# adamgreig/labrador-ldpc

Hardware: AMD Instinct MI355X
Metric: decoded codewords/sec @25 min-sum iters, TM8192, Eb/N0=2dB; 1/2/4/8 GPU (higher is better)
Workload: dtype f32; 1 GPU; TM8192 f32 LLRs, 4194304 frames on 1 GPU = BASELINE config 4 whole, resident in HBM, max_iters 25 with early termination, AWGN Eb/N0 2.0 dB, 256 random codewords; code=TM8192, total_frames=4194304, frames_per_gpu=4194304, max_iters=25, parallelism=1 contiguous shard(s) of one batch, one process per GPU, no collective, kernel_variant=0, library_build=bc9a2135c5c5dfc7

## Files before the change

### labrador_ldpc_amd/csrc/decode_ms_pair.hpp

```cpp
#pragma once

#include "decode_ms_kernel.hpp"


namespace ldpc {


typedef float ldpc_f2 __attribute__((ext_vector_type(2)));

template <int CODE, class T>
struct PairGeometry {
    static constexpr int M = CODES[CODE].m;
    static constexpr int NT = M / 2;
    static constexpr int NX = count_exchanged(*CODES[CODE].proto);
    static constexpr int NXC = count_exch_cols(*CODES[CODE].proto);
    static constexpr int OUT_LEN = CODES[CODE].output_len();
    static constexpr int LDS_BYTES = ((NX + NXC) * M * 4 + 16 + 15) / 16 * 16;
    static_assert(M % 512 == 0 && NT <= 1024, "pair ownership needs M/8 >= 64 lanes per quarter and <= 1024 threads");
};

constexpr int pair_local_rank(const Prototype &p, int S, int B)
{
    int nloc = 0, r = 0;
    for (int b = 0; b < p.n_blocks; ++b)
        if (blk_local(p.blk[b])) { if (b < B) ++r; ++nloc; }
    return S * nloc + r;
}

constexpr bool all_exchanged_are_pi(const Prototype &p)
{
    for (int b = 0; b < p.n_blocks; ++b)
        if (!blk_local(p.blk[b]) && p.blk[b].kind != BLK_P) return false;
    return true;
}

template <class T, bool SOFT, bool CORRECTED>
constexpr int pair_hoist_addresses()
{
    if (LDPC_PAIR_HOIST >= 0) return LDPC_PAIR_HOIST;
    return (std::is_same_v<T, float> && !SOFT && !CORRECTED) ? LDPC_PAIR_HOIST_F32 : 0;
}

template <int CODE, class T, int JW, int FORM, bool SOFT = false, bool CORRECTED = false>
LDPC_DEV void decode_ms_pair_body(const T *__restrict__ llrs, uint8_t *__restrict__ output,
                                  uint32_t *__restrict__ iters_out, uint8_t *__restrict__ success_out,
                                  uint32_t batch, uint32_t maxiters, float nocap_limit, uint32_t *claim, char *lds,
                                  T *__restrict__ app = nullptr, float corr_scale = 1.0f, float corr_offset = 0.0f)
{
    static_assert(!CORRECTED || std::is_same_v<T, float>, "the correction step is built for f32 messages");
    using GEO = PairGeometry<CODE, T>;
    using O = Ops<T>;
    using R = typename O::R;
    static_assert(sizeof(R) == 4 && sizeof(typename O::E) == 4, "pair kernel: 4-byte message types");
    constexpr Prototype P = *CODES[CODE].proto;
    static_assert(all_exchanged_are_pi(P), "pair kernel: exchanged blocks must be pi_k");
    constexpr int M = GEO::M, NT = GEO::NT, NB = P.n_blocks, NROWS = P.n_rows, NCOLS = P.n_cols;
    constexpr int N = CODES[CODE].n, NTX = N / M, NX = GEO::NX, NXC = GEO::NXC;
    constexpr int Q = M / 4, IPT = 2;
    constexpr int BLK_BYTES = M * 4, FLAG_OFF = (NX + NXC) * BLK_BYTES;
    constexpr bool ODD_B64 = LDPC_PAIR_ODD_B64 >= 0 ? LDPC_PAIR_ODD_B64 != 0 : true;
    constexpr int LOCAL_IN_VAR = LDPC_PAIR_LOCAL_IN_VAR >= 0 ? LDPC_PAIR_LOCAL_IN_VAR : (std::is_same_v<T, float> ? 10 : 8);
    constexpr int HOIST = pair_hoist_addresses<T, SOFT, CORRECTED>();
    constexpr bool PRIO_WAVES = true;
    (void)PRIO_WAVES;

    const int t = (int)(threadIdx.x & (M / 8 - 1)) + JW * (M / 8);
    __builtin_assume(t >= 0 && t < NT);
    const uint32_t n_groups = batch;
    uint32_t cw = blockIdx.x;
    bool live = cw < batch;
    (void)live;

    auto lds1 = [&](int off) LDPC_INLINE -> float & { return *reinterpret_cast<float *>(lds + off); };
    auto lds2 = [&](int off) LDPC_INLINE -> ldpc_f2 & { return *reinterpret_cast<ldpc_f2 *>(lds + off); };
    auto flag_at = [&](uint32_t which) LDPC_INLINE -> int & { return *reinterpret_cast<int *>(lds + FLAG_OFF + 4 * (which & 1)); };
    auto cap_flag = [&]() LDPC_INLINE -> int & { return *reinterpret_cast<int *>(lds + FLAG_OFF + 8); };
    constexpr bool NOCAP_POSSIBLE = LDPC_PAIR_NOCAP && std::is_same_v<T, float>;

    auto even_c = [](int B) constexpr { return (phi_of(P.blk[B].val, JW, M) & 1) == 0; };
    auto wire = [&](auto B_, auto S_, int tb8) LDPC_INLINE -> int {
        constexpr int B = decltype(B_)::value, S = decltype(S_)::value;
        constexpr int K = P.blk[B].val;
        constexpr int base = (((theta_of(K) + JW) & 3) * Q) * 4 + lds_bias(P, B, BLK_BYTES);
        return ((tb8 + (phi_of(K, JW, M) + S) * 4) & (Q * 4 - 1)) | base;
    };

    R u[IPT][NB], v[IPT][NB], va[IPT][NCOLS], llr[IPT][NTX];
    T lraw[IPT][NTX];

    auto fetch_llrs = [&](uint32_t c) LDPC_INLINE {
        unsigned tu = (unsigned)t;
        asm volatile("" : "+v"(tu));
        const uint32_t cc = c < batch ? c : batch - 1;
        static_for<0, NTX>([&](auto C_) LDPC_INLINE {
            constexpr int C = decltype(C_)::value;
            const T *src = (llrs + (size_t)cc * N) + (unsigned)(C * M);
            lraw[0][C] = src[2 * tu];
            lraw[1][C] = src[2 * tu + 1];
        });
    };

    auto forget_llrs = [&]() LDPC_INLINE {
        static_for<0, IPT>([&](auto S_) LDPC_INLINE {
            static_for<0, NTX>([&](auto C_) LDPC_INLINE {
                if constexpr (sizeof(T) == 4) { T &x = lraw[decltype(S_)::value][decltype(C_)::value]; asm volatile("" : "=v"(x)); }
            });
        });
    };
    (void)forget_llrs;
    constexpr int VB_HI = 0x10000;
    int had[IPT][NB], vb[2];
    (void)had; (void)vb;
    auto hoist_addresses = [&]() LDPC_INLINE {
        int tq = t;
        asm volatile("" : "+v"(tq));
        const int tb8 = tq * 8;
        vb[0] = tb8;
        asm volatile("" : "+v"(vb[0]));
        if constexpr (FLAG_OFF > VB_HI) {
            vb[1] = tb8 + VB_HI;
            asm volatile("" : "+v"(vb[1]));
        }
        static_for<0, NB>([&](auto B_) LDPC_INLINE {
            constexpr int B = decltype(B_)::value;
            if constexpr (exch_slot(P, B) >= 0) {
                constexpr int lo = lds_bias(P, B, BLK_BYTES);
                static_assert(lds_xu_off(P, exch_slot(P, B), BLK_BYTES) - lo + 4 < 0x10000 && lds_xva_off(P, col_slot(P, P.blk[B].col), BLK_BYTES) - lo + 4 < 0x10000);
                if constexpr (even_c(B)) {
                    had[0][B] = wire(B_, IC<0>{}, tb8);
                } else if constexpr (ODD_B64) {
                    had[0][B] = wire(B_, IC<-1>{}, tb8);
                    had[1][B] = wire(B_, IC<1>{}, tb8);
                    asm volatile("" : "+v"(had[1][B]));
                } else {
                    had[0][B] = wire(B_, IC<0>{}, tb8);
                    had[1][B] = wire(B_, IC<1>{}, tb8);
                    asm volatile("" : "+v"(had[1][B]));
                }
                asm volatile("" : "+v"(had[0][B]));
            }
        });
    };
    auto own = [&](auto OFF_) LDPC_INLINE -> int {
        constexpr int off = decltype(OFF_)::value;
        if constexpr (off < VB_HI) return vb[0] + off;
        else return vb[1] + (off - VB_HI);
    };
    (void)own;

    auto begin_codeword = [&]() LDPC_INLINE {
        if constexpr (HOIST == 1) hoist_addresses();
        int tq = t;
        asm volatile("" : "+v"(tq));
        const int tb8 = tq * 8;
        static_for<0, IPT>([&](auto S_) LDPC_INLINE {
            constexpr int S = decltype(S_)::value;
            static_for<0, NB>([&](auto B_) LDPC_INLINE {
                constexpr int B = decltype(B_)::value;
                u[S][B] = O::zero();
                v[S][B] = O::zero();
            });
            static_for<0, NCOLS>([&](auto C_) LDPC_INLINE { va[S][decltype(C_)::value] = O::zero(); });
            static_for<0, NTX>([&](auto C_) LDPC_INLINE { llr[S][decltype(C_)::value] = O::load(lraw[S][decltype(C_)::value]); });
        });
        if constexpr (!LDPC_PAIR_PEEL_FIRST)
        static_for<0, NX>([&](auto X_) LDPC_INLINE {
            lds2(lds_xu_off(P, decltype(X_)::value, BLK_BYTES) + tb8) = ldpc_f2{0.0f, 0.0f};
        });
        if (t < 2) flag_at(t) = 0;
        if constexpr (NOCAP_POSSIBLE) {
            bool big = false;
            static_for<0, IPT>([&](auto S_) LDPC_INLINE {
                static_for<0, NTX>([&](auto C_) LDPC_INLINE {
                    const R a = O::mag(llr[decltype(S_)::value][decltype(C_)::value]);
                    big |= !(a <= nocap_limit) || (a != 0.0f && a < 0x1p-20f);
                });
            });
            if (__ballot(big) != 0 && (t & 63) == 0) cap_flag() = 1;
        }
    };

    auto edge_update = [&](auto S_, auto B_, R x, auto BND_) LDPC_INLINE {
        constexpr int S = decltype(S_)::value, B = decltype(B_)::value;
        const R nv = O::sub_nv(x, u[S][B]);
        constexpr bool BND = decltype(BND_)::value != 0;
        constexpr int F = (FORM >= 2 && (BND || sizeof(T) <= 2)) ? FORM : (LDPC_PAIR_SELFCORR_CARRY != 0 ? 1 : 0);
        v[S][B] = O::template self_correct_b<BND, F>(nv, v[S][B]);
    };

    auto variable_phase = [&](auto BND_, auto FIRST_) LDPC_INLINE {
        constexpr bool FIRST = decltype(FIRST_)::value != 0;
        int tq = t;
        if constexpr (HOIST == 0) asm volatile("" : "+v"(tq));
        const int tb8 = tq * 8;
        (void)tb8;
        LDPC_SETPRIO(LDPC_PRIO_VAR);
        static_for<0, NCOLS>([&](auto C_) LDPC_INLINE {
            constexpr int C = decltype(C_)::value;
            if constexpr (C == NCOLS / 2) LDPC_SETPRIO(0);
            R acc0 = O::zero(), acc1 = O::zero();
            if constexpr (C < NTX) { acc0 = llr[0][C]; acc1 = llr[1][C]; }
            if constexpr (!FIRST)
            static_for<0, NB>([&](auto B_) LDPC_INLINE {
                constexpr int B = decltype(B_)::value;
                if constexpr (P.blk[B].col == C) {
                    constexpr int slot = exch_slot(P, B);
                    if constexpr (slot >= 0) {
                        ldpc_f2 up;
                        if constexpr (HOIST != 0) up = lds2(own(IC<lds_xu_off(P, slot, BLK_BYTES)>{}));
                        else up = lds2(lds_xu_off(P, slot, BLK_BYTES) + tb8);
                        acc0 = O::add(acc0, O::from_lds(up.x));
                        acc1 = O::add(acc1, O::from_lds(up.y));
                    } else {
                        acc0 = O::add(acc0, u[0][B]);
                        acc1 = O::add(acc1, u[1][B]);
                    }
                }
            });
            va[0][C] = acc0;
            va[1][C] = acc1;
            constexpr int cs = col_slot(P, C);
            if constexpr (cs >= 0) {
                if constexpr (HOIST != 0) lds2(own(IC<lds_xva_off(P, cs, BLK_BYTES)>{})) = ldpc_f2{O::store(acc0), O::store(acc1)};
                else lds2(lds_xva_off(P, cs, BLK_BYTES) + tb8) = ldpc_f2{O::store(acc0), O::store(acc1)};
            }
        });
        static_for<0, IPT>([&](auto S_) LDPC_INLINE {
            static_for<0, NB>([&](auto B_) LDPC_INLINE {
                constexpr int S = decltype(S_)::value, B = decltype(B_)::value;
                if constexpr (exch_slot(P, B) < 0 && pair_local_rank(P, S, B) < LOCAL_IN_VAR) {
                    if constexpr (FIRST) v[S][B] = va[S][P.blk[B].col];
                    else edge_update(S_, B_, va[S][P.blk[B].col], BND_);
                }
            });
        });
    };

    auto check_phase = [&](uint32_t it, auto CAP_, auto FIRST_) LDPC_INLINE {
        constexpr bool CAP = decltype(CAP_)::value != 0;
        constexpr bool FIRST = decltype(FIRST_)::value != 0;
        constexpr int BND = (!CAP && NOCAP_POSSIBLE) ? 1 : 0;
        int par_any = 0;
        int tq = t;
        if constexpr (HOIST == 0) asm volatile("" : "+v"(tq));
        const int tb8 = tq * 8;
        (void)tb8;
        LDPC_SETPRIO(3);
        R xs[IPT][NB];
        int ad[IPT][NB];
        auto request_marginals = [&]() LDPC_INLINE {
        static_for<0, NB>([&](auto B_) LDPC_INLINE {
            constexpr int B = decltype(B_)::value;
            constexpr int slot = exch_slot(P, B);
            if constexpr (slot >= 0) {
                constexpr int cs = col_slot(P, P.blk[B].col);
                constexpr int off = lds_xva_off(P, cs, BLK_BYTES) - lds_bias(P, B, BLK_BYTES);
                if constexpr (HOIST != 0) {
                    ad[0][B] = had[0][B];
                    if constexpr (!even_c(B)) ad[1][B] = had[1][B];
                }
                if constexpr (even_c(B)) {
                    if constexpr (HOIST == 0) ad[0][B] = wire(B_, IC<0>{}, tb8);
                    const ldpc_f2 xp = lds2(off + ad[0][B]);
                    xs[0][B] = O::from_lds(xp.x);
                    xs[1][B] = O::from_lds(xp.y);
                } else if constexpr (ODD_B64) {
                    if constexpr (HOIST == 0) {
                        ad[0][B] = wire(B_, IC<-1>{}, tb8);
                        ad[1][B] = wire(B_, IC<1>{}, tb8);
                    }
                    const ldpc_f2 lo = lds2(off + ad[0][B]), hi = lds2(off + ad[1][B]);
                    xs[0][B] = O::from_lds(lo.y);
                    xs[1][B] = O::from_lds(hi.x);
                } else {
                    if constexpr (HOIST == 0) {
                        ad[0][B] = wire(B_, IC<0>{}, tb8);
                        ad[1][B] = wire(B_, IC<1>{}, tb8);
                    }
                    xs[0][B] = O::from_lds(lds1(off + ad[0][B]));
                    xs[1][B] = O::from_lds(lds1(off + ad[1][B]));
                }
            }
        });
        };
        auto local_edges = [&]() LDPC_INLINE {
        static_for<0, IPT>([&](auto S_) LDPC_INLINE {
            static_for<0, NB>([&](auto B_) LDPC_INLINE {
                constexpr int S = decltype(S_)::value, B = decltype(B_)::value;
                if constexpr (exch_slot(P, B) < 0 && pair_local_rank(P, S, B) >= LOCAL_IN_VAR) {
                    if constexpr (FIRST) v[S][B] = va[S][P.blk[B].col];
                    else edge_update(S_, B_, va[S][P.blk[B].col], IC<BND>{});
                }
            });
        });
        };
        request_marginals();
        __builtin_amdgcn_sched_barrier(0);
        local_edges();
        __builtin_amdgcn_sched_barrier(0);
        static_for<0, IPT>([&](auto S_) LDPC_INLINE {
            static_for<0, NB>([&](auto B_) LDPC_INLINE {
                constexpr int S = decltype(S_)::value, B = decltype(B_)::value;
                if constexpr (exch_slot(P, B) >= 0) {
                    if constexpr (FIRST) v[S][B] = xs[S][B];
                    else edge_update(S_, B_, xs[S][B], IC<BND>{});
                }
            });
        });
        static_for<0, NROWS>([&](auto R_) LDPC_INLINE {
            constexpr int Rw = decltype(R_)::value;
            constexpr int D = row_degree(P, Rw);
            static_for<0, IPT>([&](auto S_) LDPC_INLINE {
                constexpr int S = decltype(S_)::value;
                {
                    constexpr int prio_rows[6] = LDPC_PRIO_ROWS_PAIR;
                    constexpr int step = Rw * IPT + S, nsteps = IPT * NROWS;
                    constexpr int k = step - (nsteps - 6);
                    constexpr int now = k >= 0 ? prio_rows[k] : 3, before = (step > 0 && k >= 1) ? prio_rows[k - 1] : 3;
                    if constexpr (now != before) LDPC_SETPRIO(now);
                }
                R a[D], e[D];
                int sr[D], xw[D];
                static_for<0, D>([&](auto J_) LDPC_INLINE {
                    constexpr int J = decltype(J_)::value;
                    constexpr int B = row_block(P, Rw, J);
                    a[J] = v[S][B];
                    sr[J] = O::sign_word(v[S][B]);
                    if constexpr (exch_slot(P, B) >= 0) xw[J] = O::bits(xs[S][B]);
                    else xw[J] = O::bits(va[S][P.blk[B].col]);
                });
                const int sgn = xor_reduce<D>(sr), par = xor_reduce<D>(xw);
                exclusive_min<O, D, true, CAP>(a, e);
                if constexpr (CORRECTED)
                    static_for<0, D>([&](auto J_) LDPC_INLINE {
                        constexpr int J = decltype(J_)::value;
                        e[J] = __builtin_fmaxf(__fsub_rn(__fmul_rn(corr_scale, e[J]), corr_offset), 0.0f);
                    });
                static_for<0, D>([&](auto J_) LDPC_INLINE {
                    constexpr int J = decltype(J_)::value;
                    constexpr int B = row_block(P, Rw, J);
                    u[S][B] = O::apply_sign(e[J], sgn, sr[J]);
                    constexpr int slot = exch_slot(P, B);
                    if constexpr (slot >= 0) {
                        constexpr int off = lds_xu_off(P, slot, BLK_BYTES) - lds_bias(P, B, BLK_BYTES);
                        if constexpr (!even_c(B)) lds1(off + ad[S][B] + (ODD_B64 && S == 0 ? 4 : 0)) = O::store(u[S][B]);
                        else if constexpr (S == 1) lds2(off + ad[0][B]) = ldpc_f2{O::store(u[0][B]), O::store(u[1][B])};
                    }
                });
                par_any |= par;
            });
        });
        if (par_any < 0) flag_at(it) = 1;
    };

    if (t == 0) cap_flag() = 0;
    if constexpr (HOIST == 2) hoist_addresses();
    LDPC_SYNC();
    constexpr bool FETCH_EARLY = LDPC_PAIR_FETCH_EARLY >= 0 ? LDPC_PAIR_FETCH_EARLY != 0 : sizeof(T) >= 4;
    if (FETCH_EARLY && blockIdx.x < n_groups) fetch_llrs(blockIdx.x);
    const bool dyn = claim != nullptr && maxiters != 0;
    uint32_t ticket = 0;
    int *const next_word = reinterpret_cast<int *>(lds + FLAG_OFF + 12);
    auto collect_claim = [&]() LDPC_INLINE {
        if constexpr (JW == 0) {
            if (dyn && t == 0) {
                *next_word = (int)(gridDim.x + ticket);
                if (ticket == n_groups - 1) __hip_atomic_store(claim, 0u, __ATOMIC_RELAXED, __HIP_MEMORY_SCOPE_AGENT);
            }
        }
    };
    for (uint32_t g = blockIdx.x; g < n_groups;) {
        cw = (uint32_t)__builtin_amdgcn_readfirstlane((int)g);
        if constexpr (JW == 0) {
            if (dyn && t == 0) ticket = __hip_atomic_fetch_add(claim, 1u, __ATOMIC_RELAXED, __HIP_MEMORY_SCOPE_AGENT);
        }
        if constexpr (!FETCH_EARLY) fetch_llrs(cw);
        begin_codeword();
        bool done = false, ok = false;
        uint32_t iters = maxiters;
        auto iterate = [&](auto CAP_) LDPC_INLINE {
            uint32_t it0 = 0;
            if constexpr (LDPC_PAIR_PEEL_FIRST != 0) {
                if (maxiters == 0) { done = true; return; }
                variable_phase(IC<(decltype(CAP_)::value == 0 && NOCAP_POSSIBLE) ? 1 : 0>{}, IC<1>{});
                LDPC_SYNC();
                check_phase(0u, CAP_, IC<1>{});
                collect_claim();
                it0 = 1;
            }
            for (uint32_t it = it0;; ++it) {
                if (it > 0) LDPC_SYNC();
                if (it > 0 && flag_at(it - 1) == 0) { done = true; ok = true; iters = it - 1; }
                else if (it == maxiters) { done = true; }
                if (done) break;
                variable_phase(IC<(decltype(CAP_)::value == 0 && NOCAP_POSSIBLE) ? 1 : 0>{}, IC<0>{});
                LDPC_SYNC();
                if (it > 0 && t == 0) flag_at(it - 1) = 0;
                check_phase(it, CAP_, IC<0>{});
                if constexpr (LDPC_PAIR_PEEL_FIRST == 0) { if (it == 0) collect_claim(); }
            }
        };
        LDPC_SYNC();
        if constexpr (NOCAP_POSSIBLE) {
            if (__builtin_amdgcn_readfirstlane(cap_flag()) != 0) iterate(IC<1>{});
            else iterate(IC<0>{});
        } else {
            iterate(IC<1>{});
        }
        const uint32_t g_next = dyn ? (uint32_t)__builtin_amdgcn_readfirstlane(*next_word) : g + gridDim.x;
        if (FETCH_EARLY && g_next < n_groups) fetch_llrs(g_next);
        else if constexpr (HOIST != 0 && FETCH_EARLY && sizeof(T) == 4) forget_llrs();
        static_for<0, NCOLS>([&](auto C_) LDPC_INLINE {
            constexpr int C = decltype(C_)::value;
            const unsigned long long ev = __ballot(O::bits(va[0][C]) < 0), od = __ballot(O::bits(va[1][C]) < 0);
            unsigned long long w[2];
            static_for<0, 2>([&](auto H_) LDPC_INLINE {
                constexpr int H = decltype(H_)::value;
                unsigned long long re, ro;
                const unsigned e32 = (unsigned)(ev >> (32 * H)), o32 = (unsigned)(od >> (32 * H));
                asm("s_bitreplicate_b64_b32 %0, %1" : "=s"(re) : "s"(e32));
                asm("s_bitreplicate_b64_b32 %0, %1" : "=s"(ro) : "s"(o32));
                const unsigned long long il = (re & 0x5555555555555555ull) | (ro & 0xAAAAAAAAAAAAAAAAull);
                const unsigned lo = __builtin_bswap32(__builtin_bitreverse32((unsigned)il));
                const unsigned hi = __builtin_bswap32(__builtin_bitreverse32((unsigned)(il >> 32)));
                w[H] = (unsigned long long)lo | ((unsigned long long)hi << 32);
            });
            if constexpr (SOFT) {
                struct alignas(2 * sizeof(T)) Pair { T e, o; };
                unsigned tu = (unsigned)t;
                asm volatile("" : "+v"(tu));
                Pair *const dst_app = reinterpret_cast<Pair *>(app + (size_t)cw * (NCOLS * M) + C * M + 2 * tu);
                Pair pr{soft_value<T>(va[0][C]), soft_value<T>(va[1][C])};
                *dst_app = pr;
                if constexpr (std::is_floating_point_v<T> && C < NTX) {
                    if (__ballot(va[0][C] == __builtin_inff() || va[1][C] == __builtin_inff()) != 0) {
                        const T *src = (llrs + (size_t)cw * N) + (unsigned)(C * M) + 2 * tu;
                        const T x0 = src[0], x1 = src[1];
                        pr.e = x0 != x0 ? x0 : pr.e;
                        pr.o = x1 != x1 ? x1 : pr.o;
                        *dst_app = pr;
                    }
                }
            }
            if ((t & 63) == 0) {
                unsigned long long *dst = reinterpret_cast<unsigned long long *>((output + (size_t)cw * GEO::OUT_LEN) + (C * M + 2 * t) / 8);
                dst[0] = w[0];
                dst[1] = w[1];
            }
        });
        if (t == 0) { iters_out[cw] = iters; success_out[cw] = ok ? 1 : 0; cap_flag() = 0; }
        LDPC_SYNC();
        g = g_next;
    }
}

template <class T>
constexpr int pair_form_default()
{
    if (LDPC_PAIR_SELFCORR_MED3 >= 0) return LDPC_PAIR_SELFCORR_MED3;
    if (sizeof(T) <= 2) return 6;
    return (sizeof(T) > 4 || std::is_same_v<T, int32_t>) ? 0 : 2;
}

template <int CODE, class T, int FORM = pair_form_default<T>()>
__global__ void __launch_bounds__((PairGeometry<CODE, T>::NT))
decode_ms_pair_kernel(const T *__restrict__ llrs, uint8_t *__restrict__ output, uint32_t *__restrict__ iters_out,
                      uint8_t *__restrict__ success_out, uint32_t batch, uint32_t maxiters, float nocap_limit, uint32_t *claim)
{
    using GEO = PairGeometry<CODE, T>;
    __shared__ __attribute__((aligned(16))) char lds[GEO::LDS_BYTES];
    const int jw = __builtin_amdgcn_readfirstlane((int)threadIdx.x) / (GEO::M / 8);
    if (jw == 0) decode_ms_pair_body<CODE, T, 0, FORM>(llrs, output, iters_out, success_out, batch, maxiters, nocap_limit, claim, lds);
    else if (jw == 1) decode_ms_pair_body<CODE, T, 1, FORM>(llrs, output, iters_out, success_out, batch, maxiters, nocap_limit, claim, lds);
    else if (jw == 2) decode_ms_pair_body<CODE, T, 2, FORM>(llrs, output, iters_out, success_out, batch, maxiters, nocap_limit, claim, lds);
    else decode_ms_pair_body<CODE, T, 3, FORM>(llrs, output, iters_out, success_out, batch, maxiters, nocap_limit, claim, lds);
}

template <int CODE, class T, int FORM = pair_form_default<T>()>
__global__ void __launch_bounds__((PairGeometry<CODE, T>::NT))
soft_decode_ms_pair_kernel(const T *__restrict__ llrs, T *__restrict__ app, uint8_t *__restrict__ output, uint32_t *__restrict__ iters_out,
                           uint8_t *__restrict__ success_out, uint32_t batch, uint32_t maxiters, float nocap_limit, uint32_t *claim)
{
    using GEO = PairGeometry<CODE, T>;
    __shared__ __attribute__((aligned(16))) char lds[GEO::LDS_BYTES];
    const int jw = __builtin_amdgcn_readfirstlane((int)threadIdx.x) / (GEO::M / 8);
    if (jw == 0) decode_ms_pair_body<CODE, T, 0, FORM, true>(llrs, output, iters_out, success_out, batch, maxiters, nocap_limit, claim, lds, app);
    else if (jw == 1) decode_ms_pair_body<CODE, T, 1, FORM, true>(llrs, output, iters_out, success_out, batch, maxiters, nocap_limit, claim, lds, app);
    else if (jw == 2) decode_ms_pair_body<CODE, T, 2, FORM, true>(llrs, output, iters_out, success_out, batch, maxiters, nocap_limit, claim, lds, app);
    else decode_ms_pair_body<CODE, T, 3, FORM, true>(llrs, output, iters_out, success_out, batch, maxiters, nocap_limit, claim, lds, app);
}

}
```

### labrador_ldpc_amd/csrc/decode_ms_tuning.hpp

```cpp
#pragma once

#ifndef LDPC_TUNING_OVERRIDES_ALLOWED
#if defined(LDPC_QUARTER_SPECIALISE) || defined(LDPC_NOCAP) || defined(LDPC_LOCAL_IN_VAR) || defined(LDPC_PRIO) || defined(LDPC_PRIO_ROWS) || \
    defined(LDPC_PRIO_ROWS_LEAN) || defined(LDPC_PRIO_VAR) || defined(LDPC_TM2048_WAVES) || defined(LDPC_PAIR_LOCAL_IN_VAR) || defined(LDPC_PAIR_NOCAP) || \
    defined(LDPC_PAIR_ODD_B64) || defined(LDPC_PRIO_ROWS_PAIR) || defined(LDPC_SELFCORR_CARRY) || defined(LDPC_WAVE_VERDICT) || defined(LDPC_WG_VERDICT) || \
    defined(LDPC_PEEL_FIRST) || defined(LDPC_PAIR_PEEL_FIRST) || defined(LDPC_PAIR_FETCH_EARLY) || defined(LDPC_PAIR_SELFCORR_CARRY) || \
    defined(LDPC_SELFCORR_MED3) || defined(LDPC_PAIR_SELFCORR_MED3) || defined(LDPC_LEAN_CH) || \
    defined(LDPC_PAIR_HOIST) || defined(LDPC_PAIR_HOIST_F32)
#error "the LDPC_* tuning switches are fixed in a library build (kernel experiments: tools/kbench/)"
#endif
#endif

#ifndef LDPC_QUARTER_SPECIALISE
#define LDPC_QUARTER_SPECIALISE 2
#endif
#ifndef LDPC_SELFCORR_CARRY
#define LDPC_SELFCORR_CARRY -1
#endif
#ifndef LDPC_SELFCORR_MED3
#define LDPC_SELFCORR_MED3 -1
#endif
#ifndef LDPC_PAIR_SELFCORR_MED3
#define LDPC_PAIR_SELFCORR_MED3 -1
#endif
#ifndef LDPC_PAIR_FETCH_EARLY
#define LDPC_PAIR_FETCH_EARLY -1
#endif
#ifndef LDPC_PAIR_PEEL_FIRST
#define LDPC_PAIR_PEEL_FIRST 1
#endif
#ifndef LDPC_PAIR_SELFCORR_CARRY
#define LDPC_PAIR_SELFCORR_CARRY 0
#endif
#ifndef LDPC_WAVE_VERDICT
#define LDPC_WAVE_VERDICT 1
#endif
#ifndef LDPC_PEEL_FIRST
#define LDPC_PEEL_FIRST -1
#endif
#ifndef LDPC_WG_VERDICT
#define LDPC_WG_VERDICT -1
#endif
#ifndef LDPC_NOCAP
#define LDPC_NOCAP 1
#endif
#ifndef LDPC_LOCAL_IN_VAR
#define LDPC_LOCAL_IN_VAR -1
#endif
#ifndef LDPC_PRIO
#define LDPC_PRIO 2
#endif
#ifndef LDPC_PRIO_ROWS
#define LDPC_PRIO_ROWS {2, 2, 1, 1, 1, 0}
#endif
#ifndef LDPC_LEAN_CH
#define LDPC_LEAN_CH 6
#endif
#ifndef LDPC_PRIO_ROWS_LEAN
#define LDPC_PRIO_ROWS_LEAN {3, 3, 3, 2, 1, 0}
#endif
#ifndef LDPC_PRIO_VAR
#define LDPC_PRIO_VAR 2
#endif
#ifndef LDPC_TM2048_WAVES
#define LDPC_TM2048_WAVES 6
#endif

#ifndef LDPC_PAIR_LOCAL_IN_VAR
#define LDPC_PAIR_LOCAL_IN_VAR -1
#endif
#ifndef LDPC_PAIR_NOCAP
#define LDPC_PAIR_NOCAP 1
#endif
#ifndef LDPC_PAIR_ODD_B64
#define LDPC_PAIR_ODD_B64 -1
#endif
#ifndef LDPC_PAIR_HOIST
#define LDPC_PAIR_HOIST -1
#endif
#ifndef LDPC_PAIR_HOIST_F32
#define LDPC_PAIR_HOIST_F32 2
#endif

#ifndef LDPC_PRIO_ROWS_PAIR
#define LDPC_PRIO_ROWS_PAIR {3, 3, 2, 2, 1, 0}
#endif
```

Before: 8.839 million codewords/s.

## Issue first exchanged-message LDS reads alongside the parity flag read after barrier

In the f32 pair decoder's iteration loop, the first EARLY (default 8) exchanged u-message LDS reads of the variable phase are now issued right after the barrier, together with the early-termination flag read. They are consumed later through graded lgkmcnt waits. This hides LDS latency behind the flag check and branch. The flag double-buffer is handled by explicit offset toggling, and a full lgkmcnt(0) drain follows the loop. The cost is more live VGPRs for the prefetched values and fragile hand-written asm counting.

After: 9.307 million codewords/s, median of 6. 5.3% higher.

```diff
diff --git a/labrador_ldpc_amd/csrc/decode_ms_pair.hpp b/labrador_ldpc_amd/csrc/decode_ms_pair.hpp
--- a/labrador_ldpc_amd/csrc/decode_ms_pair.hpp
+++ b/labrador_ldpc_amd/csrc/decode_ms_pair.hpp
@@ -39,6 +39,28 @@
 {
     if (LDPC_PAIR_HOIST >= 0) return LDPC_PAIR_HOIST;
     return (std::is_same_v<T, float> && !SOFT && !CORRECTED) ? LDPC_PAIR_HOIST_F32 : 0;
+}
+
+constexpr int pair_var_read_block(const Prototype &p, int k)
+{
+    for (int c = 0; c < p.n_cols; ++c)
+        for (int b = 0; b < p.n_blocks; ++b)
+            if (p.blk[b].col == c && exch_slot(p, b) >= 0 && k-- == 0) return b;
+    return -1;
+}
+constexpr int pair_var_read_rank(const Prototype &p, int B)
+{
+    for (int k = 0; k < p.n_blocks; ++k)
+        if (pair_var_read_block(p, k) == B) return k;
+    return -1;
+}
+
+template <int HOIST, int NX>
+constexpr int pair_early_u()
+{
+    if (HOIST == 0 || LDPC_PAIR_PEEL_FIRST == 0) return 0;
+    if (LDPC_PAIR_EARLY_U >= 0) return LDPC_PAIR_EARLY_U < NX ? LDPC_PAIR_EARLY_U : NX;
+    return LDPC_PAIR_EARLY_U_F32 < NX ? LDPC_PAIR_EARLY_U_F32 : NX;
 }
 
 template <int CODE, class T, int JW, int FORM, bool SOFT = false, bool CORRECTED = false>
@@ -61,6 +83,8 @@
     constexpr bool ODD_B64 = LDPC_PAIR_ODD_B64 >= 0 ? LDPC_PAIR_ODD_B64 != 0 : true;
     constexpr int LOCAL_IN_VAR = LDPC_PAIR_LOCAL_IN_VAR >= 0 ? LDPC_PAIR_LOCAL_IN_VAR : (std::is_same_v<T, float> ? 10 : 8);
     constexpr int HOIST = pair_hoist_addresses<T, SOFT, CORRECTED>();
+    constexpr int EARLY = pair_early_u<HOIST, NX>();
+    static_assert(EARLY >= 0 && EARLY <= 15, "lgkmcnt counts to 15");
     constexpr bool PRIO_WAVES = true;
     (void)PRIO_WAVES;
 
@@ -86,6 +110,10 @@
     };
 
     R u[IPT][NB], v[IPT][NB], va[IPT][NCOLS], llr[IPT][NTX];
+    int fnext = 0;
+    (void)fnext;
+    ldpc_f2 upre[EARLY > 0 ? EARLY : 1];
+    (void)upre;
     T lraw[IPT][NTX];
 
     auto fetch_llrs = [&](uint32_t c) LDPC_INLINE {
@@ -190,6 +218,8 @@
 
     auto variable_phase = [&](auto BND_, auto FIRST_) LDPC_INLINE {
         constexpr bool FIRST = decltype(FIRST_)::value != 0;
+        constexpr bool PRE = EARLY > 0 && !FIRST;
+        (void)PRE;
         int tq = t;
         if constexpr (HOIST == 0) asm volatile("" : "+v"(tq));
         const int tb8 = tq * 8;
@@ -207,7 +237,13 @@
                     constexpr int slot = exch_slot(P, B);
                     if constexpr (slot >= 0) {
                         ldpc_f2 up;
-                        if constexpr (HOIST != 0) up = lds2(own(IC<lds_xu_off(P, slot, BLK_BYTES)>{}));
+                        constexpr int rank = pair_var_read_rank(P, B);
+                        if constexpr (PRE && rank < EARLY) {
+                            ldpc_f2 &x = upre[rank];
+                            asm volatile("s_waitcnt lgkmcnt(%1)" : "+v"(x) : "n"(EARLY - 1 - rank));
+                            up = x;
+                        }
+                        else if constexpr (HOIST != 0) up = lds2(own(IC<lds_xu_off(P, slot, BLK_BYTES)>{}));
                         else up = lds2(lds_xu_off(P, slot, BLK_BYTES) + tb8);
                         acc0 = O::add(acc0, O::from_lds(up.x));
                         acc1 = O::add(acc1, O::from_lds(up.y));
@@ -350,7 +386,8 @@
                 par_any |= par;
             });
         });
-        if (par_any < 0) flag_at(it) = 1;
+        if constexpr (EARLY > 0 && !FIRST) { if (par_any < 0) *reinterpret_cast<int *>(lds + fnext) = 1; }
+        else if (par_any < 0) flag_at(it) = 1;
     };
 
     if (t == 0) cap_flag() = 0;
@@ -388,6 +425,35 @@
                 collect_claim();
                 it0 = 1;
             }
+            if constexpr (EARLY > 0) {
+                int fsel = FLAG_OFF;
+                for (uint32_t it = 1;; ++it) {
+                    asm volatile("" : "+s"(it));
+                    LDPC_SYNC();
+                    int fl, fa;
+                    asm volatile("" : "+s"(fsel));
+                    asm volatile("v_mov_b32 %0, %2\n\tds_read_b32 %1, %0" : "=&v"(fa), "=v"(fl) : "s"(fsel));
+                    static_for<0, EARLY>([&](auto K_) LDPC_INLINE {
+                        constexpr int K = decltype(K_)::value;
+                        constexpr int off = lds_xu_off(P, exch_slot(P, pair_var_read_block(P, K)), BLK_BYTES);
+                        static_assert((off < VB_HI ? off : off - VB_HI) < 0x10000);
+                        ldpc_f2 &x = upre[K];
+                        const int &base = vb[off < VB_HI ? 0 : 1];
+                        asm volatile("ds_read_b64 %0, %1 offset:%2" : "=v"(x) : "v"(base), "n"(off < VB_HI ? off : off - VB_HI));
+                    });
+                    asm volatile("s_waitcnt lgkmcnt(%1)" : "+v"(fl) : "n"(EARLY));
+                    if (__builtin_amdgcn_readfirstlane(fl) == 0) { done = true; ok = true; iters = it - 1; }
+                    else if (it == maxiters) { done = true; }
+                    if (done) break;
+                    variable_phase(IC<(decltype(CAP_)::value == 0 && NOCAP_POSSIBLE) ? 1 : 0>{}, IC<0>{});
+                    LDPC_SYNC();
+                    if (t == 0) *reinterpret_cast<int *>(lds + fa) = 0;
+                    fsel ^= 4;
+                    asm volatile("" : "+s"(fsel));
+                    fnext = fsel;
+                    check_phase(it, CAP_, IC<0>{});
+                }
+            } else
             for (uint32_t it = it0;; ++it) {
                 if (it > 0) LDPC_SYNC();
                 if (it > 0 && flag_at(it - 1) == 0) { done = true; ok = true; iters = it - 1; }
@@ -406,6 +472,10 @@
             else iterate(IC<0>{});
         } else {
             iterate(IC<1>{});
+        }
+        if constexpr (EARLY > 0) {
+            asm volatile("s_waitcnt lgkmcnt(0)");
+            __builtin_amdgcn_sched_barrier(0);
         }
         const uint32_t g_next = dyn ? (uint32_t)__builtin_amdgcn_readfirstlane(*next_word) : g + gridDim.x;
         if (FETCH_EARLY && g_next < n_groups) fetch_llrs(g_next);
diff --git a/labrador_ldpc_amd/csrc/decode_ms_tuning.hpp b/labrador_ldpc_amd/csrc/decode_ms_tuning.hpp
--- a/labrador_ldpc_amd/csrc/decode_ms_tuning.hpp
+++ b/labrador_ldpc_amd/csrc/decode_ms_tuning.hpp
@@ -6,7 +6,7 @@
     defined(LDPC_PAIR_ODD_B64) || defined(LDPC_PRIO_ROWS_PAIR) || defined(LDPC_SELFCORR_CARRY) || defined(LDPC_WAVE_VERDICT) || defined(LDPC_WG_VERDICT) || \
     defined(LDPC_PEEL_FIRST) || defined(LDPC_PAIR_PEEL_FIRST) || defined(LDPC_PAIR_FETCH_EARLY) || defined(LDPC_PAIR_SELFCORR_CARRY) || \
     defined(LDPC_SELFCORR_MED3) || defined(LDPC_PAIR_SELFCORR_MED3) || defined(LDPC_LEAN_CH) || \
-    defined(LDPC_PAIR_HOIST) || defined(LDPC_PAIR_HOIST_F32)
+    defined(LDPC_PAIR_HOIST) || defined(LDPC_PAIR_HOIST_F32) || defined(LDPC_PAIR_EARLY_U) || defined(LDPC_PAIR_EARLY_U_F32)
 #error "the LDPC_* tuning switches are fixed in a library build (kernel experiments: tools/kbench/)"
 #endif
 #endif
@@ -81,6 +81,12 @@
 #ifndef LDPC_PAIR_HOIST_F32
 #define LDPC_PAIR_HOIST_F32 2
 #endif
+#ifndef LDPC_PAIR_EARLY_U
+#define LDPC_PAIR_EARLY_U -1
+#endif
+#ifndef LDPC_PAIR_EARLY_U_F32
+#define LDPC_PAIR_EARLY_U_F32 8
+#endif
 
 #ifndef LDPC_PRIO_ROWS_PAIR
 #define LDPC_PRIO_ROWS_PAIR {3, 3, 2, 2, 1, 0}
```
